# bauerca/maxwell

Hardware: NVIDIA B200
Metric: curlcurl_spmv_crs_equiv_gbs (higher is better)
Workload: dtype f64

## Files before the change

### maxwell_b200/csrc/mxg_internal.h

```cpp
#pragma once
#include <cuda_runtime.h>
#include <nccl.h>

#include <cstdarg>
#include <cstdint>
#include <cstdio>
#include <memory>
#include <string>
#include <vector>

#include "mxgpu.h"

namespace mxg {

void setError(const char* fmt, ...);

#define MXG_CUDA(expr)                                                                       \
  do {                                                                                       \
    cudaError_t e_ = (expr);                                                                 \
    if (e_ != cudaSuccess) {                                                                 \
      mxg::setError("%s:%d: %s failed: %s", __FILE__, __LINE__, #expr, cudaGetErrorString(e_)); \
      return MXG_ERR_CUDA;                                                                   \
    }                                                                                        \
  } while (0)
// ... 111 lines not shown
  int64_t sendCount = 0, sendOffset = 0;
  int64_t recvCount = 0, recvStart = 0;
};
}

struct mxg_crs {
  mxg_ctx* ctx = nullptr;
  mxg_map *rowMap = nullptr, *domMap = nullptr;
  bool isComplex = false;
  int64_t nRows = 0, nLoc = 0, nnz = 0;
  int64_t gLo = 0, gHi = 0;
  int32_t* dRowPat = nullptr;
  int32_t* dPatOff = nullptr;
  void* dPat = nullptr;
  int64_t numPats = 0, dictRows = 0, patEntries = 0;
  int64_t nGen = 0, ellEntries = 0;
  int32_t* dGenRow = nullptr;
  int32_t* dGenLen = nullptr;
  int64_t* dSlicePtr = nullptr;
  int32_t* dCol = nullptr;
  void* dVal = nullptr;
  int64_t intBegin = 0, intEnd = 0, genIntBegin = 0, genIntEnd = 0;
  int64_t ghostRows = 0;
  std::vector<mxg::HaloPeer> peers;
  int32_t* dSendIdx = nullptr;
  int64_t sendTotal = 0;
  mutable void* dSendBuf = nullptr;
  mutable void* dGhost = nullptr;
  mutable int haloCols = 0;
  size_t deviceBytes = 0;
  void* dInvDiag = nullptr;
  int ilv = 1;
  void* dWinTiles = nullptr;
  int winR = 0;
  int winIlv = 1;
  int winMaxVec = 1;
  int64_t winTiles = 0, winValid = 0;
  int64_t winBufElems = 0;
  struct GraphEntry {
    uint64_t key;
    cudaGraphExec_t exec;
    int launches;
  };
  mutable std::vector<GraphEntry> graphs;
  struct P2P {
    bool on = false;
    bool fused = true;
    unsigned long long hostEpoch = 0;
    int capCols = 0;
    void* ghost = nullptr;
    unsigned long long* flags = nullptr;
    unsigned long long* epoch = nullptr;
    unsigned int* done = nullptr;
    void* dArgs = nullptr;
    unsigned long long* trace = nullptr;
    int npeers = 0;
    int peerRank[8];
    void* peerGhost[8];
    unsigned long long* peerFlag[8];
    int64_t remoteStart[8], remoteGTot[8];
    std::vector<void*> opened;
  };
  mutable P2P p2p;
};

namespace mxg {
template <class T>
inline ColTable<T> tableOf(const mxg_mv* mv, int first = 0, int count = -1) {
  ColTable<T> t;
  if (count < 0) count = mv->ncols - first;
  for (int j = 0; j < count; ++j) t.p[j] = static_cast<T*>(mv->col[first + j]);
// ... 17 lines not shown
```

### maxwell_b200/csrc/mxg_spmm_win.cuh

```cuda
#pragma once
#include <algorithm>
#include <climits>
#include <cstdint>
#include <vector>

namespace mxg {

constexpr int kWinThreads = 384;

struct alignas(16) WinTile {
  int32_t segLo[3];
  int32_t segLen[3];
  int32_t shift[3];
  int32_t dLo, dHi;
  int32_t valid;
  int32_t total;
  int32_t pad[3];
};
static_assert(sizeof(WinTile) == 64, "WinTile layout");

template <class Delta>
inline std::vector<WinTile> planWinTiles(const int32_t* rowPat, const int32_t* patOff, int64_t numPats, Delta delta, int64_t nRows,
                                         int64_t nLoc, int R, int align, int64_t budgetElems, int64_t* maxTotal, int64_t* validTiles) {
  const int64_t nTiles = (nRows + R - 1) / R;
  std::vector<WinTile> tiles(static_cast<size_t>(nTiles));
  std::vector<int64_t> minRow(static_cast<size_t>(numPats), 0), maxRow(static_cast<size_t>(numPats), 0);
  std::vector<int64_t> stamp(static_cast<size_t>(numPats), -1);
  std::vector<int32_t> touched;
  struct Ent { int64_t d, lo, hi; };
  std::vector<Ent> ents;
  *maxTotal = 0;
  *validTiles = 0;
  for (int64_t t = 0; t < nTiles; ++t) {
    WinTile& W = tiles[size_t(t)];
    W = WinTile{};
    W.dLo = INT_MIN;
    W.dHi = INT_MAX;
    const int64_t r0 = t * R, r1 = std::min<int64_t>(nRows, r0 + R);
    touched.clear();
    for (int64_t r = r0; r < r1; ++r) {
      const int32_t p = rowPat[r];
      if (p < 0) continue;
      if (stamp[p] != t) { stamp[p] = t; minRow[p] = maxRow[p] = r; touched.push_back(p); }
      else maxRow[p] = r;
    }
    if (touched.empty()) continue;
    ents.clear();
    for (int32_t p : touched)
      for (int32_t q = patOff[p]; q < patOff[p + 1]; ++q) {
        const int64_t d = delta(q);
        ents.push_back({d, minRow[p] + d, maxRow[p] + d + 1});
      }
    if (ents.empty()) continue;
    std::sort(ents.begin(), ents.end(), [](const Ent& a, const Ent& b) { return a.d < b.d; });
    int64_t g1 = 0, g2 = 0;
    size_t s1 = 0, s2 = 0;
    for (size_t i = 0; i + 1 < ents.size(); ++i) {
      const int64_t g = ents[i + 1].d - ents[i].d;
      if (g > g1) { g2 = g1; s2 = s1; g1 = g; s1 = i + 1; }
      else if (g > g2) { g2 = g; s2 = i + 1; }
    }
    const int64_t minGap = 64;
    if (g2 < minGap) s2 = 0;
    if (g1 < minGap) { s1 = s2; s2 = 0; }
    size_t a = s1, b = s2;
    if (a && b && a > b) std::swap(a, b);
    if (!a) { a = b; b = 0; }
    const size_t n = ents.size();
    size_t cb[4];
    int ncl;
    if (a && b) { cb[0] = 0; cb[1] = a; cb[2] = b; cb[3] = n; ncl = 3; }
    else if (a) { cb[0] = 0; cb[1] = a; cb[2] = n; ncl = 2; }
    else { cb[0] = 0; cb[1] = n; ncl = 1; }
    int cls[3];
    if (ncl == 3) { cls[0] = 0; cls[1] = 1; cls[2] = 2; W.dLo = int32_t(ents[a].d); W.dHi = int32_t(ents[b - 1].d); }
    else if (ncl == 2) { cls[0] = 1; cls[1] = 2; W.dHi = int32_t(ents[a - 1].d); }
    else cls[0] = 1;
// ... 5 lines not shown
      for (size_t i = cb[c]; i < cb[c + 1]; ++i) { lo[c] = std::min(lo[c], ents[i].lo); hi[c] = std::max(hi[c], ents[i].hi); }
      if (lo[c] < 0 || hi[c] > nLoc) ok = false;
      lo[c] = lo[c] / align * align;
      hi[c] = (hi[c] + align - 1) / align * align;
    }
    int order[3] = {0, 1, 2};
    std::sort(order, order + ncl, [&](int x, int y) { return lo[x] < lo[y]; });
    int64_t total = 0;
    int nseg = 0, segOf[3] = {0, 0, 0};
    int64_t segLo[3] = {0, 0, 0}, segHi[3] = {0, 0, 0}, segOff[3] = {0, 0, 0};
    for (int k = 0; k < ncl && ok; ++k) {
      const int c = order[k];
      if (nseg > 0 && lo[c] <= segHi[nseg - 1]) segHi[nseg - 1] = std::max(segHi[nseg - 1], hi[c]);
      else { segLo[nseg] = lo[c]; segHi[nseg] = hi[c]; ++nseg; }
      segOf[c] = nseg - 1;
    }
    for (int sgi = 0; sgi < nseg && ok; ++sgi) {
      segOff[sgi] = total;
      total += segHi[sgi] - segLo[sgi];
      W.segLo[sgi] = int32_t(segLo[sgi]);
      W.segLen[sgi] = int32_t(segHi[sgi] - segLo[sgi]);
    }
    for (int c = 0; c < ncl && ok; ++c) W.shift[cls[c]] = int32_t(segOff[segOf[c]] - segLo[segOf[c]]);
    if (!ok || total > budgetElems || total >= (int64_t(1) << 30)) {
      W = WinTile{};
      W.dLo = INT_MIN;
      W.dHi = INT_MAX;
      continue;
    }
    W.valid = 1;
    W.total = int32_t(total);
    *maxTotal = std::max<int64_t>(*maxTotal, total);
    ++*validTiles;
  }
  return tiles;
}

#ifdef __CUDACC__
__device__ __forceinline__ uint32_t smemU32(const void* p) { return static_cast<uint32_t>(__cvta_generic_to_shared(p)); }
__device__ __forceinline__ void mbarInit(uint64_t* bar, uint32_t count) {
  asm volatile("mbarrier.init.shared::cta.b64 [%0], %1;" ::"r"(smemU32(bar)), "r"(count) : "memory");
}
__device__ __forceinline__ void mbarFenceInit() {
  asm volatile("fence.mbarrier_init.release.cluster;" ::: "memory");
  asm volatile("fence.proxy.async.shared::cta;" ::: "memory");
}
__device__ __forceinline__ void mbarExpectTx(uint64_t* bar, uint32_t bytes) {
  asm volatile("mbarrier.arrive.expect_tx.shared::cta.b64 _, [%0], %1;" ::"r"(smemU32(bar)), "r"(bytes) : "memory");
}
__device__ __forceinline__ void bulkLoad(void* dstSmem, const void* srcGlobal, uint32_t bytes, uint64_t* bar) {
  asm volatile("cp.async.bulk.shared::cluster.global.mbarrier::complete_tx::bytes [%0], [%1], %2, [%3];" ::"r"(smemU32(dstSmem)),
               "l"(srcGlobal), "r"(bytes), "r"(smemU32(bar))
               : "memory");
}
__device__ __forceinline__ void mbarWait(uint64_t* bar, uint32_t parity) {
  uint32_t done;
  do {
    asm volatile(
        "{\n"
        ".reg .pred p;\n"
        "mbarrier.try_wait.parity.shared::cta.b64 p, [%1], %2;\n"
        "selp.u32 %0, 1, 0, p;\n"
        "}\n"
        : "=r"(done)
        : "r"(smemU32(bar)), "r"(parity)
        : "memory");
  } while (!done);
}
#endif

}
```

### maxwell_b200/csrc/mxg_spmv.cu

```cuda
#include <algorithm>
#include <cstdlib>
#include <cstring>
#include <unordered_map>

#include "mxg_internal.h"
#include "mxg_ilv_model.h"
#include "mxg_order.h"
#include "mxg_spmm_win.cuh"
#include "mxg_scan.cuh"

using namespace mxg;

namespace {

constexpr int kBlock = 256;

template <class T>
struct PatEntry;
template <>
struct __align__(16) PatEntry<double> {
  double v;
  int32_t d;
  int32_t pad;
};
// ... 142 lines not shown

template <class T, bool GHOST>
__device__ __forceinline__ void sellRowSimple(int64_t i, const SellArgs<T>& S, const XSource<T>& X, const ColTable<T>& Y, int nvec,
                                              const Epilogue<T>& ep) {
  const int64_t row = S.genRow[i];
  if (row < 0) return;
  const int len = S.genLen[i];
  const int64_t base = S.slicePtr[i >> 5] + (i & 31);
  for (int j = 0; j < nvec; ++j) {
    T acc = zeroOf<T>();
    for (int k = 0; k < len; ++k) accum(acc, S.val[base + int64_t(k) * 32], loadX<T, GHOST>(X, j, S.col[base + int64_t(k) * 32]));
    storeY(Y.p[j], row, acc, ep);
  }
}

template <class T, bool GHOST, int NV>
__global__ void __launch_bounds__(kBlock) k_spmm_dict(int64_t rowBegin, int64_t rowEnd, DictArgs<T> D,
                                                      XSource<T> X, ColTable<T> Y, int nvec, Epilogue<T> ep) {
  const int64_t row = rowBegin + blockIdx.x * int64_t(kBlock) + threadIdx.x;
  if (row < rowEnd) dictRow<T, GHOST, NV>(row, D, X, Y, nvec, ep);
}

constexpr int kBlockIlv = 384;
template <class T, bool GHOST, int NV>
__global__ void __launch_bounds__(kBlockIlv) k_spmm_dict_ilv3(int64_t rowBegin, int64_t rowEnd, DictArgs<T> D,
                                                              XSource<T> X, ColTable<T> Y, int nvec, Epilogue<T> ep) {
  const int warp = threadIdx.x >> 5, lane = threadIdx.x & 31;
  const int64_t row = rowBegin + blockIdx.x * int64_t(kBlockIlv) + (warp / 3) * 96 + 3 * lane + (warp % 3);
  if (row < rowEnd) dictRow<T, GHOST, NV>(row, D, X, Y, nvec, ep);
}


template <class T>
__device__ __forceinline__ void winIssue(const WinTile& W, const T* __restrict__ xcol, T* buf, uint64_t* bar) {
  uint32_t bytes = 0;
#pragma unroll
  for (int sgi = 0; sgi < 3; ++sgi) bytes += uint32_t(W.segLen[sgi]) * uint32_t(sizeof(T));
  mbarExpectTx(bar, bytes);
  int off = 0;
#pragma unroll
  for (int sgi = 0; sgi < 3; ++sgi) {
    if (W.segLen[sgi] > 0) bulkLoad(buf + off, xcol + W.segLo[sgi], uint32_t(W.segLen[sgi]) * uint32_t(sizeof(T)), bar);
    off += W.segLen[sgi];
  }
}

constexpr int kWinSlot = 16;

template <class T>
__device__ __forceinline__ PatEntry<T> ldEntry(const PatEntry<T>* p) {
  PatEntry<T> e;
  const int4* s = reinterpret_cast<const int4*>(p);
  int4* d = reinterpret_cast<int4*>(&e);
#pragma unroll
  for (int i = 0; i < int(sizeof(PatEntry<T>) / 16); ++i) d[i] = s[i];
  return e;
}

struct WinShift {
  int32_t dLo, dHi, s0, s1, s2;
};
template <class T>
__device__ __forceinline__ T winRowDot(const PatEntry<T>* __restrict__ ent, int32_t len, int32_t r, const T* __restrict__ xs, const WinShift& w) {
  T acc = zeroOf<T>();
  int32_t q = 0;
  for (; q + 1 < len; q += 2) {
    const PatEntry<T> e0 = ldEntry<T>(ent + q);
    const PatEntry<T> e1 = ldEntry<T>(ent + q + 1);
    const T x0 = xs[r + e0.d + (e0.d < w.dLo ? w.s0 : (e0.d > w.dHi ? w.s2 : w.s1))];
    const T x1 = xs[r + e1.d + (e1.d < w.dLo ? w.s0 : (e1.d > w.dHi ? w.s2 : w.s1))];
    accum(acc, entryVal(e0), x0);
    accum(acc, entryVal(e1), x1);
  }
  if (q < len) {
    const PatEntry<T> e0 = ldEntry<T>(ent + q);
    accum(acc, entryVal(e0), xs[r + e0.d + (e0.d < w.dLo ? w.s0 : (e0.d > w.dHi ? w.s2 : w.s1))]);
  }
  return acc;
}

template <class T, int ILV, int RPT>
__global__ void __launch_bounds__(kWinThreads) k_spmm_win(int64_t rowBegin, int64_t rowEnd, int64_t tile0, DictArgs<T> D,
                                                          const WinTile* __restrict__ tiles, XSource<T> X, ColTable<T> Y, int nvec,
                                                          Epilogue<T> ep) {
  extern __shared__ __align__(128) unsigned char smemRaw[];
  uint64_t* bar = reinterpret_cast<uint64_t*>(smemRaw);
  WinTile* Ws = reinterpret_cast<WinTile*>(smemRaw + 64);
  PatEntry<T>* slots = reinterpret_cast<PatEntry<T>*>(smemRaw + 128);
  constexpr int kWarps = kWinThreads / 32;
  T* buf = reinterpret_cast<T*>(smemRaw + 128 + sizeof(PatEntry<T>) * kWarps * RPT * kWinSlot);
  constexpr int R = kWinThreads * RPT;
  const int64_t tile = tile0 + blockIdx.x;
  if (threadIdx.x == 0) {
    const int4* src = reinterpret_cast<const int4*>(tiles + tile);
    int4* dst = reinterpret_cast<int4*>(Ws);
#pragma unroll
    for (int i = 0; i < 4; ++i) dst[i] = __ldg(src + i);
    mbarInit(bar, 1);
    mbarFenceInit();
    if (Ws->valid) winIssue<T>(*Ws, X.x.p[0], buf, bar);
  }
  const int warp = threadIdx.x >> 5, lane = threadIdx.x & 31;
  const int tOff = ILV == 3 ? (warp / 3) * 96 + 3 * lane + (warp % 3) : int(threadIdx.x);
  int64_t row[RPT];
  int32_t o[RPT], len[RPT];
  bool uni[RPT];
#pragma unroll
  for (int i = 0; i < RPT; ++i) {
    row[i] = tile * R + i * kWinThreads + tOff;
    int32_t p = -1;
    if (row[i] >= rowBegin && row[i] < rowEnd) p = D.rowPat[row[i]];
    o[i] = len[i] = 0;
    if (p >= 0) { o[i] = __ldg(D.patOff + p); len[i] = __ldg(D.patOff + p + 1) - o[i]; }
    const int32_t pmax = __reduce_max_sync(0xffffffffu, p);
    uni[i] = __all_sync(0xffffffffu, p < 0 || p == pmax) && pmax >= 0;
    const int32_t oU = __shfl_sync(0xffffffffu, o[i], __ffs(__ballot_sync(0xffffffffu, p == pmax)) - 1);
    const int32_t lenU = __shfl_sync(0xffffffffu, len[i], __ffs(__ballot_sync(0xffffffffu, p == pmax)) - 1);
    uni[i] = uni[i] && lenU <= kWinSlot;
    if (uni[i] && lane < lenU) slots[(warp * RPT + i) * kWinSlot + lane] = ldEntry<T>(D.pat + oU + lane);
  }
  __syncthreads();
  if (!Ws->valid) {
#pragma unroll
    for (int i = 0; i < RPT; ++i)
      if (row[i] >= rowBegin && row[i] < rowEnd) dictRow<T, false, 1>(row[i], D, X, Y, nvec, ep);
    return;
  }
  const int32_t dLo = Ws->dLo, dHi = Ws->dHi, s0 = Ws->shift[0], s1 = Ws->shift[1], s2 = Ws->shift[2];
  for (int j = 0; j < nvec; ++j) {
    mbarWait(bar, j & 1);
    const T* __restrict__ xs = buf;
#pragma unroll
    for (int i = 0; i < RPT; ++i) {
      if (len[i] == 0) continue;
      const int32_t r = int32_t(row[i]);
      const WinShift ws{dLo, dHi, s0, s1, s2};
      const T acc = uni[i] ? winRowDot<T>(slots + (warp * RPT + i) * kWinSlot, len[i], r, xs, ws)
                           : winRowDot<T>(D.pat + o[i], len[i], r, xs, ws);
      storeY(Y.p[j], row[i], acc, ep);
    }
    if (j + 1 < nvec) {
      __syncthreads();
      if (threadIdx.x == 0) winIssue<T>(*Ws, X.x.p[j + 1], buf, bar);
    }
  }
}

template <class T, bool GHOST, int NV>
__global__ void __launch_bounds__(kBlock) k_spmm_sell(int64_t genBegin, int64_t genEnd, SellArgs<T> S,
                                                      XSource<T> X, ColTable<T> Y, int nvec, Epilogue<T> ep) {
  const int64_t i = genBegin + blockIdx.x * int64_t(kBlock) + threadIdx.x;
  if (i < genEnd) sellRow<T, GHOST, NV>(i, S, X, Y, nvec, ep);
}

struct Segments {
  int64_t begin[4], end[4];
  int blockStart[5];
};
struct WaitArgs {
  int n;
  const unsigned long long* flags;
  const unsigned long long* epoch;
  int senderRank[8];
  int* err;
  long long timeoutTicks;
};
__device__ __forceinline__ void haloWait(const WaitArgs& W, int k) {
  const unsigned long long e = *W.epoch;
  const volatile unsigned long long* f = W.flags + W.senderRank[k];
  const long long t0 = clock64();
  while (*f < e) {
    if (W.timeoutTicks > 0 && clock64() - t0 > W.timeoutTicks) {
      *W.err = 1;
      __threadfence_system();
      asm volatile("trap;");
    }
    __nanosleep(64);
  }
// ... 30 lines not shown

template <class T>
DictArgs<T> dictArgs(const mxg_crs* A) { return {A->dRowPat, A->dPatOff, static_cast<const PatEntry<T>*>(A->dPat)}; }
template <class T>
SellArgs<T> sellArgs(const mxg_crs* A) { return {A->dGenRow, A->dGenLen, A->dSlicePtr, A->dCol, static_cast<const T*>(A->dVal)}; }

template <class T, bool GHOST>
int launchSegments(const mxg_crs* A, const int64_t b[4], const int64_t e[4], const XSource<T>& X, const ColTable<T>& Y, int nvec,
                   const Epilogue<T>& ep, cudaStream_t st, const WaitArgs& W) {
  mxg_ctx* ctx = A->ctx;
  Segments G;
  int blocks = 0;
  for (int sgm = 0; sgm < 4; ++sgm) {
    G.begin[sgm] = b[sgm];
    G.end[sgm] = e[sgm] > b[sgm] ? e[sgm] : b[sgm];
    G.blockStart[sgm] = blocks;
    blocks += int((G.end[sgm] - G.begin[sgm] + kBlock - 1) / kBlock);
  }
  G.blockStart[4] = blocks;
  if (blocks == 0) return MXG_OK;
  const DictArgs<T> D = dictArgs<T>(A);
  const SellArgs<T> S = sellArgs<T>(A);
  if (nvec == 1) k_spmm_multi<T, GHOST, 1><<<blocks, kBlock, 0, st>>>(G, D, S, X, Y, nvec, ep, W);
  else if (nvec == 2) k_spmm_multi<T, GHOST, 2><<<blocks, kBlock, 0, st>>>(G, D, S, X, Y, nvec, ep, W);
  else k_spmm_multi<T, GHOST, 4><<<blocks, kBlock, 0, st>>>(G, D, S, X, Y, nvec, ep, W);
  LAUNCH_CHECK(ctx);
  return MXG_OK;
}


template <class T> struct WinCfg;
template <> struct WinCfg<double> { static constexpr int RPT = 2; };
template <> struct WinCfg<zd> { static constexpr int RPT = 1; };
constexpr size_t kWinSmemMax = 200 * 1024;
constexpr size_t kWinBufBudget = 100 * 1024;
template <class T>
constexpr size_t winSmemHeader() { return 128 + sizeof(PatEntry<T>) * (kWinThreads / 32) * WinCfg<T>::RPT * kWinSlot; }

template <class T>
int launchWin(const mxg_crs* A, int64_t rowBegin, int64_t rowEnd, const XSource<T>& X, const ColTable<T>& Y, int nvec,
              const Epilogue<T>& ep, cudaStream_t st) {
  mxg_ctx* ctx = A->ctx;
  constexpr int RPT = WinCfg<T>::RPT;
  const int R = A->winR;
  const int64_t tile0 = rowBegin / R, tiles = (rowEnd + R - 1) / R - tile0;
  const size_t smem = winSmemHeader<T>() + size_t(A->winBufElems) * sizeof(T);
  const DictArgs<T> D = dictArgs<T>(A);
  const WinTile* wt = static_cast<const WinTile*>(A->dWinTiles);
  static bool attrSet[2] = {false, false};
  if (A->winIlv == 3) {
    auto kern = k_spmm_win<T, 3, RPT>;
    if (!attrSet[0]) { MXG_CUDA(cudaFuncSetAttribute(kern, cudaFuncAttributeMaxDynamicSharedMemorySize, int(kWinSmemMax))); attrSet[0] = true; }
    kern<<<unsigned(tiles), kWinThreads, smem, st>>>(rowBegin, rowEnd, tile0, D, wt, X, Y, nvec, ep);
  } else {
    auto kern = k_spmm_win<T, 1, RPT>;
    if (!attrSet[1]) { MXG_CUDA(cudaFuncSetAttribute(kern, cudaFuncAttributeMaxDynamicSharedMemorySize, int(kWinSmemMax))); attrSet[1] = true; }
    kern<<<unsigned(tiles), kWinThreads, smem, st>>>(rowBegin, rowEnd, tile0, D, wt, X, Y, nvec, ep);
  }
  LAUNCH_CHECK(ctx);
  return MXG_OK;
}

template <class T, bool GHOST>
int launchRange(const mxg_crs* A, int64_t rowBegin, int64_t rowEnd, int64_t genBegin, int64_t genEnd, const XSource<T>& X,
                const ColTable<T>& Y, int nvec, const Epilogue<T>& ep, cudaStream_t st = nullptr) {
  mxg_ctx* ctx = A->ctx;
  if (!st) st = ctx->stream;
  const bool prof = ctx->profiling;
  if (prof) MXG_CUDA(cudaEventRecord(ctx->prof[1], ctx->stream));
  if (A->dictRows > 0 && rowEnd > rowBegin && A->winR > 0 && nvec <= A->winMaxVec) {
    const int rc = launchWin<T>(A, rowBegin, rowEnd, X, Y, nvec, ep, st);
    if (rc) return rc;
  } else if (A->dictRows > 0 && rowEnd > rowBegin) {
    const DictArgs<T> D = dictArgs<T>(A);
    if (A->ilv == 3) {
      const int64_t blocks = (rowEnd - rowBegin + kBlockIlv - 1) / kBlockIlv;
      if (nvec == 1) k_spmm_dict_ilv3<T, GHOST, 1><<<blocks, kBlockIlv, 0, st>>>(rowBegin, rowEnd, D, X, Y, nvec, ep);
      else if (nvec == 2) k_spmm_dict_ilv3<T, GHOST, 2><<<blocks, kBlockIlv, 0, st>>>(rowBegin, rowEnd, D, X, Y, nvec, ep);
      else k_spmm_dict_ilv3<T, GHOST, 4><<<blocks, kBlockIlv, 0, st>>>(rowBegin, rowEnd, D, X, Y, nvec, ep);
    } else {
      const int64_t blocks = (rowEnd - rowBegin + kBlock - 1) / kBlock;
      if (nvec == 1) k_spmm_dict<T, GHOST, 1><<<blocks, kBlock, 0, st>>>(rowBegin, rowEnd, D, X, Y, nvec, ep);
      else if (nvec == 2) k_spmm_dict<T, GHOST, 2><<<blocks, kBlock, 0, st>>>(rowBegin, rowEnd, D, X, Y, nvec, ep);
      else k_spmm_dict<T, GHOST, 4><<<blocks, kBlock, 0, st>>>(rowBegin, rowEnd, D, X, Y, nvec, ep);
    }
    LAUNCH_CHECK(ctx);
  }
  if (prof) MXG_CUDA(cudaEventRecord(ctx->prof[2], ctx->stream));
  if (genEnd > genBegin) {
    const int64_t blocks = (genEnd - genBegin + kBlock - 1) / kBlock;
    const SellArgs<T> S = sellArgs<T>(A);
// ... 548 lines not shown
  }
  int64_t covered = 0;
  for (const Peer& p : A->peers) covered += p.recvCount;
  MXG_REQUIRE(covered == int64_t(ghosts.size()), "mxg_crs_create: %lld ghost columns have no owner",
              (long long)(int64_t(ghosts.size()) - covered));
  A->sendTotal = int64_t(sendIdx.size());
  int rcU = uploadVec(sendIdx, &A->dSendIdx, &A->deviceBytes, ctx);
  if (rcU) return rcU;
  return setupP2P(A, int64_t(ghosts.size()));
}

template <class T>
int planKernels(mxg_crs* A, const std::vector<int32_t>& rowPat, const std::vector<int32_t>& patOff, const std::vector<PatEntry<T>>& pat) {
  mxg_ctx* ctx = A->ctx;
  const int64_t nRows = A->nRows, nLoc = A->nLoc;
  int rc = MXG_OK;
  {
    const char* env = std::getenv("MXG_SPMV_ILV");
    const std::string mode = env ? env : "auto";
    A->ilv = 1;
    if (mode == "3") A->ilv = 3;
    else if (mode != "1" && A->dictRows > 0) {
      const PatEntry<T>* pe = pat.data();
      const mxg::IlvCost cost = mxg::ilvCostModel(rowPat.data(), patOff.data(), [pe](int32_t q) { return pe[q].d; }, A->intBegin,
                                                  A->intEnd, int(sizeof(T)), int(sizeof(PatEntry<T>)));
      if (mxg::ilvWins(cost)) A->ilv = 3;
    }
  }

  {
    const char* env = std::getenv("MXG_SPMV_WIN");
    const bool want = !(env && std::strcmp(env, "0") == 0);
    if (want && A->dictRows > 0 && nLoc + A->gLo + A->gHi < (int64_t(1) << 30)) {
      constexpr int R = kWinThreads * WinCfg<T>::RPT;
      constexpr int align = 16 / int(sizeof(T)) > 0 ? 16 / int(sizeof(T)) : 1;
      const PatEntry<T>* pe = pat.data();
      int64_t maxTotal = 0, valid = 0;
      std::vector<WinTile> tiles = planWinTiles(rowPat.data(), patOff.data(), A->numPats, [pe](int32_t q) { return int64_t(pe[q].d); }, nRows,
                                                nLoc, R, align, int64_t(std::min(kWinBufBudget, kWinSmemMax - winSmemHeader<T>()) / sizeof(T)), &maxTotal, &valid);
      if (valid > 0) {
        WinTile* dT = nullptr;
        if ((rc = uploadVec(tiles, &dT, &A->deviceBytes, ctx))) return rc;
        A->dWinTiles = dT;
        A->winR = R;
        A->winTiles = int64_t(tiles.size());
        A->winValid = valid;
        A->winBufElems = maxTotal;
        A->winMaxVec = 1;
        if (const char* mv = std::getenv("MXG_WIN_MAXVEC")) A->winMaxVec = std::atoi(mv);
        int64_t same1 = 0, same3 = 0;
        for (int64_t r = 0; r + 3 < nRows; ++r) {
          if (rowPat[r] < 0) continue;
          same1 += rowPat[r] == rowPat[r + 1];
          same3 += rowPat[r] == rowPat[r + 3];
        }
        A->winIlv = same3 > same1 ? 3 : 1;
        if (const char* iv = std::getenv("MXG_SPMV_ILV")) {
          if (std::strcmp(iv, "1") == 0) A->winIlv = 1;
          if (std::strcmp(iv, "3") == 0) A->winIlv = 3;
        }
      }
    }
  }

  return rc;
}

template <class T>
int buildImpl(mxg_crs* A, const int64_t* rowptr, const int64_t* colGids, const double* valsIn, int layout) {
  mxg_ctx* ctx = A->ctx;
  constexpr int w = sizeof(T) / sizeof(double);
  const T* vals = reinterpret_cast<const T*>(valsIn);
  const int64_t nRows = A->nRows, nLoc = A->nLoc;
  const int64_t nnzIn = rowptr[nRows];
  const mxg_map* dom = A->domMap;
  MXG_REQUIRE(dom->nGlobal < (int64_t(1) << 31), "mxg_crs_create: global size must fit in 31 bits");

  std::vector<int32_t> lookup(size_t(dom->nGlobal), -1);
  for (int64_t i = 0; i < nLoc; ++i) lookup[dom->gids[i]] = int32_t(i);
  const int64_t domLo = nLoc ? dom->gids.front() : 0, domHi = nLoc ? dom->gids.back() : -1;
// ... 713 lines not shown
  domain_map->refs++;
  A->isComplex = is_complex != 0;
  A->nRows = row_map->nLocal;
  A->nLoc = domain_map->nLocal;
  int rc = A->isComplex ? buildImpl<zd>(A, rowptr, col_gids, vals, layout) : buildImpl<double>(A, rowptr, col_gids, vals, layout);
  if (rc) {
    mxg_crs_destroy(A);
    return rc;
  }
  *out = A;
  return MXG_OK;
}

int mxg_crs_create(mxg_map* row_map, mxg_map* domain_map, const int64_t* rowptr, const int64_t* col_gids,
                   const double* vals, int is_complex, mxg_crs** out) {
  int layout = 0;
  if (const char* e = std::getenv("MXG_SPMV_LAYOUT")) layout = (std::strcmp(e, "sell") == 0) ? 1 : 0;
  return mxg_crs_create_opts(row_map, domain_map, rowptr, col_gids, vals, is_complex, layout, out);
}

int mxg_crs_destroy(mxg_crs* A) {
  if (!A) return MXG_OK;
  cudaSetDevice(A->ctx->device);
  cudaStreamSynchronize(A->ctx->stream);
  cudaStreamSynchronize(A->ctx->commStream);
  for (auto& g : A->graphs) cudaGraphExecDestroy(g.exec);
  for (void* o : A->p2p.opened) cudaIpcCloseMemHandle(o);
  if (A->p2p.ghost) cudaFree(A->p2p.ghost);
  if (A->p2p.flags) cudaFree(A->p2p.flags);
  if (A->p2p.epoch) cudaFree(A->p2p.epoch);
  if (A->p2p.done) cudaFree(A->p2p.done);
  if (A->p2p.trace) cudaFree(A->p2p.trace);
  if (A->p2p.dArgs) cudaFree(A->p2p.dArgs);
  void* ptrs[] = {A->dRowPat, A->dPatOff, A->dPat, A->dGenRow, A->dGenLen, A->dSlicePtr, A->dCol, A->dVal, A->dSendIdx, A->dSendBuf, A->dGhost, A->dInvDiag, A->dWinTiles};
  for (void* p : ptrs)
    if (p) cudaFree(p);
  mxg_map_destroy(A->rowMap);
  mxg_map_destroy(A->domMap);
  delete A;
  return MXG_OK;
}

static int checkApply(const char* fn, const mxg_crs* A, const mxg_mv* x, const mxg_mv* y) {
  MXG_REQUIRE(A && x && y, "%s: NULL argument", fn);
  MXG_REQUIRE(x->map->ctx == A->ctx && y->map->ctx == A->ctx, "%s: operands live on different contexts", fn);
  MXG_REQUIRE(x->isComplex == A->isComplex && y->isComplex == A->isComplex, "%s: mixed real/complex operands", fn);
  MXG_REQUIRE(x->ld == A->nLoc, "%s: x has local length %lld, operator domain has %lld", fn, (long long)x->ld, (long long)A->nLoc);
  MXG_REQUIRE(y->ld == A->nRows, "%s: y has local length %lld, operator range has %lld", fn, (long long)y->ld, (long long)A->nRows);
  MXG_REQUIRE(x->ncols == y->ncols, "%s: x has %d columns, y has %d", fn, x->ncols, y->ncols);
  if (x->storage.get() == y->storage.get())
    for (void* px : x->col)
      for (void* py : y->col) MXG_REQUIRE(px != py, "%s: x and y must not alias", fn);
  return MXG_OK;
}

int mxg_crs_apply(const mxg_crs* A, const mxg_mv* x, mxg_mv* y) {
  int rc = checkApply("mxg_crs_apply", A, x, y);
  if (rc) return rc;
  MXG_CUDA(cudaSetDevice(A->ctx->device));
  if (A->isComplex) {
    Epilogue<zd> ep{{1, 0}, {0, 0}, 0};
    return applyImpl<zd>(A, x, y, ep);
  }
  Epilogue<double> ep{1.0, 0.0, 0};
  return applyImpl<double>(A, x, y, ep);
}

// ... 140 lines not shown
```

Before: 15470.

## Make windowed SpMM persistent with a warp-specialized TMA producer ring

Converts the windowed SpMM kernel from one CTA per tile into a persistent grid. A dedicated producer warp streams tile descriptors, x windows, per-tile pattern entry lists and per-row slot bytes into a multi-stage mbarrier ring using bulk async copies. Consumer warps compute rows from shared-memory pattern entries with unrolled multi-row dot products and write y through shared buffers with bulk stores. The aim is to overlap loads with compute and to cut global dictionary gathers. The cost is more host-side planning, extra device arrays, higher shared-memory use, and more complex synchronization.

```diff
diff --git a/maxwell_b200/csrc/mxg_internal.h b/maxwell_b200/csrc/mxg_internal.h
--- a/maxwell_b200/csrc/mxg_internal.h
+++ b/maxwell_b200/csrc/mxg_internal.h
@@ -167,11 +167,14 @@
   void* dInvDiag = nullptr;
   int ilv = 1;
   void* dWinTiles = nullptr;
+  uint8_t* dWinSlot = nullptr;
+  void* dWinList = nullptr;
   int winR = 0;
   int winIlv = 1;
   int winMaxVec = 1;
   int64_t winTiles = 0, winValid = 0;
   int64_t winBufElems = 0;
+  int64_t winEntElems = 0;
   struct GraphEntry {
     uint64_t key;
     cudaGraphExec_t exec;
diff --git a/maxwell_b200/csrc/mxg_spmm_win.cuh b/maxwell_b200/csrc/mxg_spmm_win.cuh
--- a/maxwell_b200/csrc/mxg_spmm_win.cuh
+++ b/maxwell_b200/csrc/mxg_spmm_win.cuh
@@ -1,36 +1,60 @@
 #pragma once
 #include <algorithm>
 #include <climits>
+#include <map>
 #include <cstdint>
 #include <vector>
 
+#ifdef __CUDACC__
+#define MXG_WIN_HD __host__ __device__
+#else
+#define MXG_WIN_HD
+#endif
+
 namespace mxg {
 
-constexpr int kWinThreads = 384;
+constexpr int kWinConsumerWarps = 12;
+constexpr int kWinConsumers = 32 * kWinConsumerWarps;
+constexpr int kWinThreads = kWinConsumers + 32;
+constexpr int kWinMaxPats = 15;
+constexpr int kWinMaxEnt = 240;
+constexpr uint8_t kSlotNone = 0xFF;
+constexpr uint8_t kSlotGlobal = 0xFE;
 
 struct alignas(16) WinTile {
   int32_t segLo[3];
   int32_t segLen[3];
   int32_t shift[3];
   int32_t dLo, dHi;
-  int32_t valid;
   int32_t total;
-  int32_t pad[3];
+  int32_t listOff;
+  uint8_t entBase[kWinMaxPats + 1];
+  uint8_t valid;
+  uint8_t nPat;
+  uint8_t overCap;
+  uint8_t pad;
+  int32_t pad2[2];
 };
-static_assert(sizeof(WinTile) == 64, "WinTile layout");
+static_assert(sizeof(WinTile) == 80, "WinTile layout");
 
 template <class Delta>
 inline std::vector<WinTile> planWinTiles(const int32_t* rowPat, const int32_t* patOff, int64_t numPats, Delta delta, int64_t nRows,
-                                         int64_t nLoc, int R, int align, int64_t budgetElems, int64_t* maxTotal, int64_t* validTiles) {
+                                         int64_t nLoc, int R, int align, int64_t budgetElems, int64_t* maxTotal, int64_t* validTiles,
+                                         std::vector<uint8_t>* slots, std::vector<int32_t>* lists, int64_t* maxEnt) {
   const int64_t nTiles = (nRows + R - 1) / R;
   std::vector<WinTile> tiles(static_cast<size_t>(nTiles));
   std::vector<int64_t> minRow(static_cast<size_t>(numPats), 0), maxRow(static_cast<size_t>(numPats), 0);
-  std::vector<int64_t> stamp(static_cast<size_t>(numPats), -1);
-  std::vector<int32_t> touched;
+  std::vector<int64_t> stamp(static_cast<size_t>(numPats), -1), uses(static_cast<size_t>(numPats), 0);
+  std::vector<int32_t> slotOf(static_cast<size_t>(numPats), kSlotGlobal);
+  std::vector<int32_t> touched, key;
+  std::map<std::vector<int32_t>, int32_t> listAt;
+  lists->clear();
   struct Ent { int64_t d, lo, hi; };
   std::vector<Ent> ents;
+  slots->assign(static_cast<size_t>(nTiles * R), kSlotNone);
   *maxTotal = 0;
   *validTiles = 0;
+  *maxEnt = 0;
   for (int64_t t = 0; t < nTiles; ++t) {
     WinTile& W = tiles[size_t(t)];
     W = WinTile{};
@@ -41,8 +65,9 @@
     for (int64_t r = r0; r < r1; ++r) {
       const int32_t p = rowPat[r];
       if (p < 0) continue;
-      if (stamp[p] != t) { stamp[p] = t; minRow[p] = maxRow[p] = r; touched.push_back(p); }
+      if (stamp[p] != t) { stamp[p] = t; minRow[p] = maxRow[p] = r; uses[p] = 0; touched.push_back(p); }
       else maxRow[p] = r;
+      ++uses[p];
     }
     if (touched.empty()) continue;
     ents.clear();
@@ -114,9 +139,54 @@
     W.total = int32_t(total);
     *maxTotal = std::max<int64_t>(*maxTotal, total);
     ++*validTiles;
+    std::stable_sort(touched.begin(), touched.end(), [&](int32_t x, int32_t y) { return uses[x] > uses[y]; });
+    int nPat = 0, nEnt = 0;
+    for (int32_t p : touched) {
+      const int len = patOff[p + 1] - patOff[p];
+      if (nPat < kWinMaxPats && nEnt + len <= kWinMaxEnt) {
+        key.push_back(p);
+        W.entBase[nPat] = uint8_t(nEnt);
+        slotOf[p] = nPat++;
+        nEnt += len;
+      } else {
+        slotOf[p] = kSlotGlobal;
+        W.overCap = 1;
+      }
+    }
+    W.nPat = uint8_t(nPat);
+    W.entBase[nPat] = uint8_t(nEnt);
+    const auto it = listAt.find(key);
+    if (it != listAt.end()) W.listOff = it->second;
+    else {
+      W.listOff = int32_t(lists->size());
+      listAt.emplace(key, W.listOff);
+      for (int32_t p : key)
+        for (int32_t q = patOff[p]; q < patOff[p + 1]; ++q) lists->push_back(q);
+    }
+    key.clear();
+    *maxEnt = std::max<int64_t>(*maxEnt, nEnt);
+    for (int64_t r = r0; r < r1; ++r)
+      if (rowPat[r] >= 0) (*slots)[size_t(r)] = uint8_t(slotOf[rowPat[r]]);
   }
   return tiles;
 }
+
+template <class Delta>
+inline std::vector<WinTile> planWinTiles(const int32_t* rowPat, const int32_t* patOff, int64_t numPats, Delta delta, int64_t nRows,
+                                         int64_t nLoc, int R, int align, int64_t budgetElems, int64_t* maxTotal, int64_t* validTiles) {
+  std::vector<uint8_t> slots;
+  std::vector<int32_t> lists;
+  int64_t maxEnt = 0;
+  return planWinTiles(rowPat, patOff, numPats, delta, nRows, nLoc, R, align, budgetElems, maxTotal, validTiles, &slots, &lists, &maxEnt);
+}
+
+MXG_WIN_HD inline void winItemRange(int64_t items, int64_t grid, int64_t b, int64_t* first, int64_t* count) {
+  const int64_t lo = items * b / grid, hi = items * (b + 1) / grid;
+  *first = lo;
+  *count = hi - lo;
+}
+MXG_WIN_HD inline uint32_t winFullParity(int64_t k, int S) { return uint32_t((k / S) & 1); }
+MXG_WIN_HD inline uint32_t winEmptyParity(int64_t k, int S) { return uint32_t((k / S - 1) & 1); }
 
 #ifdef __CUDACC__
 __device__ __forceinline__ uint32_t smemU32(const void* p) { return static_cast<uint32_t>(__cvta_generic_to_shared(p)); }
@@ -149,6 +219,19 @@
         : "memory");
   } while (!done);
 }
+__device__ __forceinline__ void mbarArrive(uint64_t* bar) {
+  asm volatile("mbarrier.arrive.shared::cta.b64 _, [%0];" ::"r"(smemU32(bar)) : "memory");
+}
+__device__ __forceinline__ void bulkStore(void* dstGlobal, const void* srcSmem, uint32_t bytes) {
+  asm volatile("cp.async.bulk.global.shared::cta.bulk_group [%0], [%1], %2;" ::"l"(dstGlobal), "r"(smemU32(srcSmem)), "r"(bytes)
+               : "memory");
+}
+__device__ __forceinline__ void bulkCommit() { asm volatile("cp.async.bulk.commit_group;" ::: "memory"); }
+template <int N>
+__device__ __forceinline__ void bulkWaitRead() { asm volatile("cp.async.bulk.wait_group.read %0;" ::"n"(N) : "memory"); }
+__device__ __forceinline__ void bulkWait0() { asm volatile("cp.async.bulk.wait_group 0;" ::: "memory"); }
+__device__ __forceinline__ void fenceProxyAsyncShared() { asm volatile("fence.proxy.async.shared::cta;" ::: "memory"); }
+__device__ __forceinline__ void namedBarrier(int id, int threads) { asm volatile("bar.sync %0, %1;" ::"r"(id), "r"(threads) : "memory"); }
 #endif
 
 }
diff --git a/maxwell_b200/csrc/mxg_spmv.cu b/maxwell_b200/csrc/mxg_spmv.cu
--- a/maxwell_b200/csrc/mxg_spmv.cu
+++ b/maxwell_b200/csrc/mxg_spmv.cu
@@ -198,22 +198,6 @@
 
 
 template <class T>
-__device__ __forceinline__ void winIssue(const WinTile& W, const T* __restrict__ xcol, T* buf, uint64_t* bar) {
-  uint32_t bytes = 0;
-#pragma unroll
-  for (int sgi = 0; sgi < 3; ++sgi) bytes += uint32_t(W.segLen[sgi]) * uint32_t(sizeof(T));
-  mbarExpectTx(bar, bytes);
-  int off = 0;
-#pragma unroll
-  for (int sgi = 0; sgi < 3; ++sgi) {
-    if (W.segLen[sgi] > 0) bulkLoad(buf + off, xcol + W.segLo[sgi], uint32_t(W.segLen[sgi]) * uint32_t(sizeof(T)), bar);
-    off += W.segLen[sgi];
-  }
-}
-
-constexpr int kWinSlot = 16;
-
-template <class T>
 __device__ __forceinline__ PatEntry<T> ldEntry(const PatEntry<T>* p) {
   PatEntry<T> e;
   const int4* s = reinterpret_cast<const int4*>(p);
@@ -225,91 +209,212 @@
 
 struct WinShift {
   int32_t dLo, dHi, s0, s1, s2;
+  __device__ __forceinline__ int32_t of(int32_t d) const { return d < dLo ? s0 : (d > dHi ? s2 : s1); }
 };
-template <class T>
-__device__ __forceinline__ T winRowDot(const PatEntry<T>* __restrict__ ent, int32_t len, int32_t r, const T* __restrict__ xs, const WinShift& w) {
+constexpr int kWinUnroll = 4;
+template <class T, int N>
+__device__ __forceinline__ void winRowsDot(const PatEntry<T>* __restrict__ ent, int32_t len, const int32_t (&r)[N], const T* __restrict__ xs,
+                                           const WinShift& w, T (&acc)[N]) {
+  int32_t q = 0;
+  for (; q + kWinUnroll <= len; q += kWinUnroll) {
+    PatEntry<T> e[kWinUnroll];
+    T xv[kWinUnroll][N];
+#pragma unroll
+    for (int u = 0; u < kWinUnroll; ++u) e[u] = ldEntry<T>(ent + q + u);
+#pragma unroll
+    for (int u = 0; u < kWinUnroll; ++u) {
+      const int32_t c = e[u].d + w.of(e[u].d);
+#pragma unroll
+      for (int i = 0; i < N; ++i) xv[u][i] = xs[r[i] + c];
+    }
+#pragma unroll
+    for (int u = 0; u < kWinUnroll; ++u)
+#pragma unroll
+      for (int i = 0; i < N; ++i) accum(acc[i], entryVal(e[u]), xv[u][i]);
+  }
+  for (; q < len; ++q) {
+    const PatEntry<T> e0 = ldEntry<T>(ent + q);
+    const int32_t c0 = e0.d + w.of(e0.d);
+#pragma unroll
+    for (int i = 0; i < N; ++i) accum(acc[i], entryVal(e0), xs[r[i] + c0]);
+  }
+}
+
+template <class T>
+__device__ __forceinline__ T gatherRowDot(const DictArgs<T>& D, const T* __restrict__ x, int64_t row, int32_t p) {
+  const int32_t o = __ldg(D.patOff + p), oe = __ldg(D.patOff + p + 1);
   T acc = zeroOf<T>();
-  int32_t q = 0;
-  for (; q + 1 < len; q += 2) {
-    const PatEntry<T> e0 = ldEntry<T>(ent + q);
-    const PatEntry<T> e1 = ldEntry<T>(ent + q + 1);
-    const T x0 = xs[r + e0.d + (e0.d < w.dLo ? w.s0 : (e0.d > w.dHi ? w.s2 : w.s1))];
-    const T x1 = xs[r + e1.d + (e1.d < w.dLo ? w.s0 : (e1.d > w.dHi ? w.s2 : w.s1))];
-    accum(acc, entryVal(e0), x0);
-    accum(acc, entryVal(e1), x1);
-  }
-  if (q < len) {
-    const PatEntry<T> e0 = ldEntry<T>(ent + q);
-    accum(acc, entryVal(e0), xs[r + e0.d + (e0.d < w.dLo ? w.s0 : (e0.d > w.dHi ? w.s2 : w.s1))]);
+  for (int32_t q = o; q < oe; ++q) {
+    const PatEntry<T> e = D.pat[q];
+    accum(acc, entryVal(e), ldgT(x + row + e.d));
   }
   return acc;
 }
 
+template <class T>
+__device__ __forceinline__ T epiValue(const T* y, int64_t row, T acc, const Epilogue<T>& ep) {
+  if (ep.mode == 0) return acc;
+  if (isZero(ep.beta)) return ep.alpha * acc;
+  return ep.alpha * acc + ep.beta * y[row];
+}
+
+constexpr int kWinMaxStages = 4;
+constexpr int kWinYBufs = 3;
+struct WinRing {
+  int S;
+  uint32_t stageBytes, xOff, entOff, slotOff, ringOff;
+};
+
 template <class T, int ILV, int RPT>
-__global__ void __launch_bounds__(kWinThreads) k_spmm_win(int64_t rowBegin, int64_t rowEnd, int64_t tile0, DictArgs<T> D,
-                                                          const WinTile* __restrict__ tiles, XSource<T> X, ColTable<T> Y, int nvec,
-                                                          Epilogue<T> ep) {
+__global__ void __launch_bounds__(kWinThreads, 2) k_spmm_win(int64_t rowBegin, int64_t rowEnd, int64_t tile0, int64_t items, WinRing ring,
+                                                          DictArgs<T> D, const WinTile* __restrict__ tiles, const uint8_t* __restrict__ slots,
+                                                          const PatEntry<T>* __restrict__ lists, XSource<T> X, ColTable<T> Y, int nvec, Epilogue<T> ep) {
   extern __shared__ __align__(128) unsigned char smemRaw[];
-  uint64_t* bar = reinterpret_cast<uint64_t*>(smemRaw);
-  WinTile* Ws = reinterpret_cast<WinTile*>(smemRaw + 64);
-  PatEntry<T>* slots = reinterpret_cast<PatEntry<T>*>(smemRaw + 128);
-  constexpr int kWarps = kWinThreads / 32;
-  T* buf = reinterpret_cast<T*>(smemRaw + 128 + sizeof(PatEntry<T>) * kWarps * RPT * kWinSlot);
-  constexpr int R = kWinThreads * RPT;
-  const int64_t tile = tile0 + blockIdx.x;
+  constexpr int R = kWinConsumers * RPT;
+  const int S = ring.S;
+  uint64_t* full = reinterpret_cast<uint64_t*>(smemRaw);
+  uint64_t* empty = full + kWinMaxStages;
+  T* ybuf = reinterpret_cast<T*>(smemRaw + 128);
+  unsigned char* stage0 = smemRaw + ring.ringOff;
+  int64_t first, count;
+  winItemRange(items, gridDim.x, blockIdx.x, &first, &count);
   if (threadIdx.x == 0) {
-    const int4* src = reinterpret_cast<const int4*>(tiles + tile);
-    int4* dst = reinterpret_cast<int4*>(Ws);
-#pragma unroll
-    for (int i = 0; i < 4; ++i) dst[i] = __ldg(src + i);
-    mbarInit(bar, 1);
+    for (int s = 0; s < S; ++s) {
+      mbarInit(full + s, 1);
+      mbarInit(empty + s, kWinConsumerWarps);
+    }
     mbarFenceInit();
-    if (Ws->valid) winIssue<T>(*Ws, X.x.p[0], buf, bar);
-  }
+  }
+  __syncthreads();
   const int warp = threadIdx.x >> 5, lane = threadIdx.x & 31;
+
+  if (warp == kWinConsumerWarps) {
+    if (lane != 0) return;
+    constexpr int kDesc = int(sizeof(WinTile) / 16);
+    int4 next[kDesc];
+#pragma unroll
+    for (int i = 0; i < kDesc; ++i) next[i] = __ldg(reinterpret_cast<const int4*>(tiles + tile0 + first / nvec) + i);
+    for (int64_t k = 0; k < count; ++k) {
+      const int s = int(k % S);
+      if (k >= S) mbarWait(empty + s, winEmptyParity(k, S));
+      const int64_t item = first + k, tile = tile0 + item / nvec;
+      const int j = int(item % nvec);
+      unsigned char* st = stage0 + size_t(s) * ring.stageBytes;
+      WinTile* Ws = reinterpret_cast<WinTile*>(st);
+#pragma unroll
+      for (int i = 0; i < kDesc; ++i) reinterpret_cast<int4*>(Ws)[i] = next[i];
+      if (k + 1 < count) {
+        const int4* src = reinterpret_cast<const int4*>(tiles + tile0 + (item + 1) / nvec);
+#pragma unroll
+        for (int i = 0; i < kDesc; ++i) next[i] = __ldg(src + i);
+      }
+      const T* xcol = X.x.p[j];
+      if (reinterpret_cast<uintptr_t>(xcol) & 15) Ws->valid = 0;
+      if (!Ws->valid) {
+        mbarArrive(full + s);
+        continue;
+      }
+      const int nPat = Ws->nPat;
+      uint32_t bytes = uint32_t(Ws->entBase[nPat]) * uint32_t(sizeof(PatEntry<T>)) + uint32_t(R);
+#pragma unroll
+      for (int sgi = 0; sgi < 3; ++sgi) bytes += uint32_t(Ws->segLen[sgi]) * uint32_t(sizeof(T));
+      mbarExpectTx(full + s, bytes);
+      T* xs = reinterpret_cast<T*>(st + ring.xOff);
+      int off = 0;
+#pragma unroll
+      for (int sgi = 0; sgi < 3; ++sgi) {
+        if (Ws->segLen[sgi] > 0) bulkLoad(xs + off, xcol + Ws->segLo[sgi], uint32_t(Ws->segLen[sgi]) * uint32_t(sizeof(T)), full + s);
+        off += Ws->segLen[sgi];
+      }
+      if (Ws->entBase[nPat] > 0)
+        bulkLoad(st + ring.entOff, lists + Ws->listOff, uint32_t(Ws->entBase[nPat]) * uint32_t(sizeof(PatEntry<T>)), full + s);
+      bulkLoad(st + ring.slotOff, slots + tile * R, uint32_t(R), full + s);
+    }
+    return;
+  }
+
   const int tOff = ILV == 3 ? (warp / 3) * 96 + 3 * lane + (warp % 3) : int(threadIdx.x);
-  int64_t row[RPT];
-  int32_t o[RPT], len[RPT];
-  bool uni[RPT];
-#pragma unroll
-  for (int i = 0; i < RPT; ++i) {
-    row[i] = tile * R + i * kWinThreads + tOff;
-    int32_t p = -1;
-    if (row[i] >= rowBegin && row[i] < rowEnd) p = D.rowPat[row[i]];
-    o[i] = len[i] = 0;
-    if (p >= 0) { o[i] = __ldg(D.patOff + p); len[i] = __ldg(D.patOff + p + 1) - o[i]; }
-    const int32_t pmax = __reduce_max_sync(0xffffffffu, p);
-    uni[i] = __all_sync(0xffffffffu, p < 0 || p == pmax) && pmax >= 0;
-    const int32_t oU = __shfl_sync(0xffffffffu, o[i], __ffs(__ballot_sync(0xffffffffu, p == pmax)) - 1);
-    const int32_t lenU = __shfl_sync(0xffffffffu, len[i], __ffs(__ballot_sync(0xffffffffu, p == pmax)) - 1);
-    uni[i] = uni[i] && lenU <= kWinSlot;
-    if (uni[i] && lane < lenU) slots[(warp * RPT + i) * kWinSlot + lane] = ldEntry<T>(D.pat + oU + lane);
-  }
-  __syncthreads();
-  if (!Ws->valid) {
-#pragma unroll
-    for (int i = 0; i < RPT; ++i)
-      if (row[i] >= rowBegin && row[i] < rowEnd) dictRow<T, false, 1>(row[i], D, X, Y, nvec, ep);
-    return;
-  }
-  const int32_t dLo = Ws->dLo, dHi = Ws->dHi, s0 = Ws->shift[0], s1 = Ws->shift[1], s2 = Ws->shift[2];
-  for (int j = 0; j < nvec; ++j) {
-    mbarWait(bar, j & 1);
-    const T* __restrict__ xs = buf;
+  for (int64_t k = 0; k < count; ++k) {
+    const int s = int(k % S);
+    const int64_t item = first + k, tile = tile0 + item / nvec;
+    const int j = int(item % nvec);
+    const unsigned char* st = stage0 + size_t(s) * ring.stageBytes;
+    const WinTile* Ws = reinterpret_cast<const WinTile*>(st);
+    mbarWait(full + s, winFullParity(k, S));
+    const int64_t tRow0 = tile * R;
+    T* __restrict__ y = Y.p[j];
+    const bool valid = Ws->valid;
+    const bool bulk = valid && tRow0 >= rowBegin && tRow0 + R <= rowEnd && !(reinterpret_cast<uintptr_t>(y + tRow0) & 15);
+    int64_t row[RPT];
+    int32_t r32[RPT];
+    bool has[RPT];
+    T acc[RPT];
 #pragma unroll
     for (int i = 0; i < RPT; ++i) {
-      if (len[i] == 0) continue;
-      const int32_t r = int32_t(row[i]);
-      const WinShift ws{dLo, dHi, s0, s1, s2};
-      const T acc = uni[i] ? winRowDot<T>(slots + (warp * RPT + i) * kWinSlot, len[i], r, xs, ws)
-                           : winRowDot<T>(D.pat + o[i], len[i], r, xs, ws);
-      storeY(Y.p[j], row[i], acc, ep);
-    }
-    if (j + 1 < nvec) {
-      __syncthreads();
-      if (threadIdx.x == 0) winIssue<T>(*Ws, X.x.p[j + 1], buf, bar);
-    }
-  }
+      row[i] = tRow0 + i * kWinConsumers + tOff;
+      r32[i] = int32_t(row[i]);
+      acc[i] = zeroOf<T>();
+    }
+    if (valid) {
+      const WinShift ws{Ws->dLo, Ws->dHi, Ws->shift[0], Ws->shift[1], Ws->shift[2]};
+      const T* __restrict__ xs = reinterpret_cast<const T*>(st + ring.xOff);
+      const PatEntry<T>* __restrict__ ents = reinterpret_cast<const PatEntry<T>*>(st + ring.entOff);
+      int slot[RPT];
+      bool same = true;
+#pragma unroll
+      for (int i = 0; i < RPT; ++i) {
+        slot[i] = row[i] >= rowBegin && row[i] < rowEnd ? st[ring.slotOff + i * kWinConsumers + tOff] : kSlotNone;
+        has[i] = slot[i] != kSlotNone;
+        same = same && slot[i] == slot[0];
+      }
+      if (same && slot[0] < kSlotGlobal) {
+        const int b = Ws->entBase[slot[0]];
+        winRowsDot<T, RPT>(ents + b, Ws->entBase[slot[0] + 1] - b, r32, xs, ws, acc);
+      } else {
+#pragma unroll
+        for (int i = 0; i < RPT; ++i) {
+          const int32_t ri[1] = {r32[i]};
+          T ai[1] = {zeroOf<T>()};
+          if (slot[i] < kSlotGlobal) {
+            const int b = Ws->entBase[slot[i]];
+            winRowsDot<T, 1>(ents + b, Ws->entBase[slot[i] + 1] - b, ri, xs, ws, ai);
+          } else if (slot[i] == kSlotGlobal) {
+            const int32_t p = D.rowPat[row[i]];
+            const int32_t o = __ldg(D.patOff + p);
+            winRowsDot<T, 1>(D.pat + o, __ldg(D.patOff + p + 1) - o, ri, xs, ws, ai);
+          }
+          acc[i] = ai[0];
+        }
+      }
+    } else {
+      const T* __restrict__ x = X.x.p[j];
+#pragma unroll
+      for (int i = 0; i < RPT; ++i) {
+        const int32_t p = row[i] >= rowBegin && row[i] < rowEnd ? D.rowPat[row[i]] : -1;
+        has[i] = p >= 0;
+        if (has[i]) acc[i] = gatherRowDot<T>(D, x, row[i], p);
+      }
+    }
+    __syncwarp();
+    if (lane == 0) mbarArrive(empty + s);
+    T* yb = ybuf + int(k % kWinYBufs) * R;
+    if (bulk) {
+#pragma unroll
+      for (int i = 0; i < RPT; ++i) yb[i * kWinConsumers + tOff] = has[i] ? epiValue(y, row[i], acc[i], ep) : y[row[i]];
+      fenceProxyAsyncShared();
+    } else {
+#pragma unroll
+      for (int i = 0; i < RPT; ++i)
+        if (has[i]) storeY(y, row[i], acc[i], ep);
+    }
+    if (threadIdx.x == 0) bulkWaitRead<kWinYBufs - 2>();
+    namedBarrier(1, kWinConsumers);
+    if (threadIdx.x == 0) {
+      if (bulk) bulkStore(y + tRow0, yb, uint32_t(R) * uint32_t(sizeof(T)));
+      bulkCommit();
+    }
+  }
+  if (threadIdx.x == 0) bulkWait0();
 }
 
 template <class T, bool GHOST, int NV>
@@ -406,10 +511,27 @@
 template <class T> struct WinCfg;
 template <> struct WinCfg<double> { static constexpr int RPT = 2; };
 template <> struct WinCfg<zd> { static constexpr int RPT = 1; };
-constexpr size_t kWinSmemMax = 200 * 1024;
+constexpr size_t kWinSmemMax = 227 * 1024;
 constexpr size_t kWinBufBudget = 100 * 1024;
-template <class T>
-constexpr size_t winSmemHeader() { return 128 + sizeof(PatEntry<T>) * (kWinThreads / 32) * WinCfg<T>::RPT * kWinSlot; }
+constexpr uint32_t alignUp(size_t v, size_t a) { return uint32_t((v + a - 1) / a * a); }
+template <class T>
+WinRing winRing(int64_t xElems, int64_t entElems) {
+  constexpr int R = kWinConsumers * WinCfg<T>::RPT;
+  WinRing g;
+  g.ringOff = alignUp(128 + kWinYBufs * size_t(R) * sizeof(T), 128);
+  g.xOff = sizeof(WinTile);
+  g.entOff = g.xOff + alignUp(size_t(xElems) * sizeof(T), 16);
+  g.slotOff = g.entOff + uint32_t(entElems) * uint32_t(sizeof(PatEntry<T>));
+  g.stageBytes = alignUp(g.slotOff + size_t(R), 128);
+  g.S = int(std::min<size_t>(kWinMaxStages, (kWinSmemMax - g.ringOff) / g.stageBytes));
+  return g;
+}
+template <class T>
+int64_t winBudgetElems() {
+  const WinRing g = winRing<T>(0, kWinMaxEnt);
+  const size_t twoStages = (kWinSmemMax - g.ringOff) / 2 - 128;
+  return int64_t(std::min(kWinBufBudget, twoStages - g.stageBytes) / sizeof(T));
+}
 
 template <class T>
 int launchWin(const mxg_crs* A, int64_t rowBegin, int64_t rowEnd, const XSource<T>& X, const ColTable<T>& Y, int nvec,
@@ -417,20 +539,23 @@
   mxg_ctx* ctx = A->ctx;
   constexpr int RPT = WinCfg<T>::RPT;
   const int R = A->winR;
-  const int64_t tile0 = rowBegin / R, tiles = (rowEnd + R - 1) / R - tile0;
-  const size_t smem = winSmemHeader<T>() + size_t(A->winBufElems) * sizeof(T);
+  const int64_t tile0 = rowBegin / R, tiles = (rowEnd + R - 1) / R - tile0, items = tiles * nvec;
+  const WinRing ring = winRing<T>(A->winBufElems, A->winEntElems);
+  const size_t smem = ring.ringOff + size_t(ring.S) * ring.stageBytes;
   const DictArgs<T> D = dictArgs<T>(A);
   const WinTile* wt = static_cast<const WinTile*>(A->dWinTiles);
-  static bool attrSet[2] = {false, false};
-  if (A->winIlv == 3) {
-    auto kern = k_spmm_win<T, 3, RPT>;
-    if (!attrSet[0]) { MXG_CUDA(cudaFuncSetAttribute(kern, cudaFuncAttributeMaxDynamicSharedMemorySize, int(kWinSmemMax))); attrSet[0] = true; }
-    kern<<<unsigned(tiles), kWinThreads, smem, st>>>(rowBegin, rowEnd, tile0, D, wt, X, Y, nvec, ep);
-  } else {
-    auto kern = k_spmm_win<T, 1, RPT>;
-    if (!attrSet[1]) { MXG_CUDA(cudaFuncSetAttribute(kern, cudaFuncAttributeMaxDynamicSharedMemorySize, int(kWinSmemMax))); attrSet[1] = true; }
-    kern<<<unsigned(tiles), kWinThreads, smem, st>>>(rowBegin, rowEnd, tile0, D, wt, X, Y, nvec, ep);
-  }
+  auto kern = A->winIlv == 3 ? k_spmm_win<T, 3, RPT> : k_spmm_win<T, 1, RPT>;
+  static int cached[2][2] = {{-1, 0}, {-1, 0}};
+  int* c = cached[A->winIlv == 3];
+  if (c[0] != int(smem)) {
+    MXG_CUDA(cudaFuncSetAttribute(kern, cudaFuncAttributeMaxDynamicSharedMemorySize, int(kWinSmemMax)));
+    MXG_CUDA(cudaOccupancyMaxActiveBlocksPerMultiprocessor(&c[1], kern, kWinThreads, smem));
+    MXG_REQUIRE(c[1] > 0, "windowed SpMM: %zu bytes of shared memory per CTA do not fit an SM", smem);
+    c[0] = int(smem);
+  }
+  const int64_t grid = std::min<int64_t>(items, int64_t(ctx->numSMs) * c[1]);
+  kern<<<unsigned(grid), kWinThreads, smem, st>>>(rowBegin, rowEnd, tile0, items, ring, D, wt, A->dWinSlot,
+                                                  static_cast<const PatEntry<T>*>(A->dWinList), X, Y, nvec, ep);
   LAUNCH_CHECK(ctx);
   return MXG_OK;
 }
@@ -1045,20 +1170,29 @@
     const char* env = std::getenv("MXG_SPMV_WIN");
     const bool want = !(env && std::strcmp(env, "0") == 0);
     if (want && A->dictRows > 0 && nLoc + A->gLo + A->gHi < (int64_t(1) << 30)) {
-      constexpr int R = kWinThreads * WinCfg<T>::RPT;
+      constexpr int R = kWinConsumers * WinCfg<T>::RPT;
       constexpr int align = 16 / int(sizeof(T)) > 0 ? 16 / int(sizeof(T)) : 1;
       const PatEntry<T>* pe = pat.data();
-      int64_t maxTotal = 0, valid = 0;
+      int64_t maxTotal = 0, valid = 0, maxEnt = 0;
+      std::vector<uint8_t> slots;
+      std::vector<int32_t> lists;
       std::vector<WinTile> tiles = planWinTiles(rowPat.data(), patOff.data(), A->numPats, [pe](int32_t q) { return int64_t(pe[q].d); }, nRows,
-                                                nLoc, R, align, int64_t(std::min(kWinBufBudget, kWinSmemMax - winSmemHeader<T>()) / sizeof(T)), &maxTotal, &valid);
+                                                nLoc, R, align, winBudgetElems<T>(), &maxTotal, &valid, &slots, &lists, &maxEnt);
       if (valid > 0) {
         WinTile* dT = nullptr;
         if ((rc = uploadVec(tiles, &dT, &A->deviceBytes, ctx))) return rc;
         A->dWinTiles = dT;
+        if ((rc = uploadVec(slots, &A->dWinSlot, &A->deviceBytes, ctx))) return rc;
+        std::vector<PatEntry<T>> listEnt(lists.size());
+        for (size_t i = 0; i < lists.size(); ++i) listEnt[i] = pat[size_t(lists[i])];
+        PatEntry<T>* dL = nullptr;
+        if ((rc = uploadVec(listEnt, &dL, &A->deviceBytes, ctx))) return rc;
+        A->dWinList = dL;
         A->winR = R;
         A->winTiles = int64_t(tiles.size());
         A->winValid = valid;
         A->winBufElems = maxTotal;
+        A->winEntElems = maxEnt;
         A->winMaxVec = 1;
         if (const char* mv = std::getenv("MXG_WIN_MAXVEC")) A->winMaxVec = std::atoi(mv);
         int64_t same1 = 0, same3 = 0;
@@ -1838,7 +1972,7 @@
   if (A->p2p.done) cudaFree(A->p2p.done);
   if (A->p2p.trace) cudaFree(A->p2p.trace);
   if (A->p2p.dArgs) cudaFree(A->p2p.dArgs);
-  void* ptrs[] = {A->dRowPat, A->dPatOff, A->dPat, A->dGenRow, A->dGenLen, A->dSlicePtr, A->dCol, A->dVal, A->dSendIdx, A->dSendBuf, A->dGhost, A->dInvDiag, A->dWinTiles};
+  void* ptrs[] = {A->dRowPat, A->dPatOff, A->dPat, A->dGenRow, A->dGenLen, A->dSlicePtr, A->dCol, A->dVal, A->dSendIdx, A->dSendBuf, A->dGhost, A->dInvDiag, A->dWinTiles, A->dWinSlot, A->dWinList};
   for (void* p : ptrs)
     if (p) cudaFree(p);
   mxg_map_destroy(A->rowMap);
```

New measurement: 8030 (median of 6 runs). 48.1% lower.
